# HKPolyU-UAV/bluerov2

Hardware: AMD Instinct MI355X
Metric: NMPC RTI solves/s (N=20, 12 states / 4 inputs), batch 4096 per GPU (higher is better)
Workload: dtype f64; 1 GPU; BASELINE.json configs[1]: batch=4096 independent BlueROV2 NMPC instances per GPU, N=20, Ts=0.05 s, circle reference window advancing one row per step, per-instance x0 noise (seed 1), nominal parameters, default options (qp_early_exit=1: exact equality-constrained shortcut when no bound is active); batch_per_gpu=4096, N=20, parallelism=single GPU

## Files before the change

bluerov2_amd/csrc/qp/fused.hpp:

```cpp
#pragma once

namespace brov {

constexpr int kFusedMaxN = 23;
template <int W, bool GRID, bool DF>
__device__ __forceinline__ bool rti_fused_step(const DevParams& P, int b, int lane, bool listed, size_t yoff) {
    extern __shared__ __attribute__((aligned(16))) double smem[];
    const int N = P.N;
    double* ba_s = smem;
    double* bv_s = ba_s + (size_t)N * kBaStage;
    double* kt_s = bv_s + (size_t)N * NX;
    double* kff_s = kt_s + (size_t)N * kKtStage;
    double* vh_s = kff_s + (size_t)N * 4;
    double* dx_s = vh_s + (size_t)N * 4;
    double* q_s = dx_s + (size_t)(N + 1) * NX;
    double* r_s = q_s + (size_t)(N + 1) * NX;
    double* const_s = r_s + (size_t)N * 4;
    if (lane == 0) { const_s[0] = 0.0; const_s[1] = 1.0; }
    LaneCst lc;
    if constexpr (W == 1) lc = load_lane_cst(P.cst, lane);
    double part = 0.0;
    bool nanp = false;
    lin_phase<W == 1, GRID>(P, b, 0, N, lane, ba_s, bv_s, kt_s, q_s, r_s, part, nanp, true, yoff);
    __syncthreads();
    if (P.dump_lin) copy_out_linearisation(P, b, 0, N, lane, ba_s, bv_s);
    std::conditional_t<GRID, InstGrid, Inst> I;
    setup_inst(P, I, b, lane, W == 1 ? &lc : nullptr, yoff);
    const bool listed_u = __builtin_amdgcn_readfirstlane((int)listed) != 0;
    I.ckpt = (N >= 8 && P.partial_refactor && listed_u) ? (N + 3) >> 2 : 0;
    I.lds_ba = (const lds_f64*)ba_s;
    I.lds_bv = (const lds_f64*)bv_s;
    I.lds_kt = (lds_f64*)kt_s;
    I.lds_q = (const lds_f64*)q_s;
    I.lds_r = (const lds_f64*)r_s;
    I.kff = kff_s;
    I.vhat = vh_s;
    I.dxb = dx_s;
    I.lds_kff = (lds_f64*)kff_s;
    I.lds_vhat = (lds_f64*)vh_s;
    I.lds_dxb = (lds_f64*)dx_s;
    I.lds_zero = (lds_f64*)const_s;
    I.lds_tr = (lds_f64*)const_s + 2;
    {
        const int rg = I.rg, cl = I.cl;
        const int zero = (int)(const_s - ba_s), one = zero + 1, kt0 = (int)(kt_s - ba_s);
        for (int r = 0; r < 3; r++) I.ba_off[r] = cl >= 3 ? (rg + 4 * r) * kBaStride + cl - 3 : ((r == 0 && rg == cl) ? one : zero);
        I.ba_str = cl >= 3 ? kBaStage : 0;
        for (int r = 0; r < 4; r++) {
            const int c = rg + 4 * r;
            I.bat_off[r] = cl >= NX ? zero : (c >= 3 ? cl * kBaStride + c - 3 : (c == cl ? one : zero));
        }
        I.bat_str = cl >= NX ? 0 : kBaStage;
        I.bat_str0 = (cl < NX && rg == 3) ? kBaStage : 0;
        for (int r = 0; r < 3; r++) I.kt_off[r] = cl < 4 ? kt0 + (rg + 4 * r) * 4 + cl : zero;
        I.kt_str = cl < 4 ? kKtStage : 0;
    }
    qp_body<W, std::conditional_t<GRID, InstGrid, Inst>, DF>(P, I, b, part, nanp);
    return I.ran_loop;
}
__device__ __forceinline__ void plant_step_wave(const DevParams& P, int b, int lane, int tk) {
    double x[NX], u[NU], k[NX], xs[NX], acc[NX];
    double* x0 = P.x0_rw + (size_t)b * NX;
#pragma unroll
    for (int j = 0; j < NX; j++) x[j] = x0[j];
#pragma unroll
    for (int j = 0; j < NU; j++) u[j] = P.res[b].u0[j];
    const ModelPar m = make_par(P.plant_pp + (size_t)b * NP);
    Wrench w = make_wrench(u);
    if (P.plant_rp) { w.k3 = P.plant_rp[(size_t)b * P.plant_rp_stride]; w.k4 = P.plant_rp[(size_t)b * P.plant_rp_stride + 1]; }
    const double h = P.plant_dt / P.plant_substeps;
    StagePoint sp;
    for (int s = 0; s < P.plant_substeps; s++) {
        model_f(x, w, m, NoWorldWrench{}, k, sp);
#pragma unroll
        for (int j = 0; j < NX; j++) { acc[j] = x[j] + (h / 6.0) * k[j]; xs[j] = x[j] + 0.5 * h * k[j]; }
        model_f(xs, w, m, NoWorldWrench{}, k, sp);
#pragma unroll
        for (int j = 0; j < NX; j++) { acc[j] += (h / 3.0) * k[j]; xs[j] = x[j] + 0.5 * h * k[j]; }
        model_f(xs, w, m, NoWorldWrench{}, k, sp);
#pragma unroll
        for (int j = 0; j < NX; j++) { acc[j] += (h / 3.0) * k[j]; xs[j] = x[j] + h * k[j]; }
        model_f(xs, w, m, NoWorldWrench{}, k, sp);
#pragma unroll
        for (int j = 0; j < NX; j++) x[j] = acc[j] + (h / 6.0) * k[j];
    }
    if (lane == 0) {
#pragma unroll
        for (int j = 0; j < NX; j++) x0[j] = x[j];
        if (P.plant_xlog) {
#pragma unroll
            for (int j = 0; j < NX; j++) P.plant_xlog[((size_t)tk * P.B + b) * NX + j] = x[j];
        }
        if (P.plant_ulog) {
#pragma unroll
            for (int j = 0; j < NU; j++) P.plant_ulog[((size_t)tk * P.B + b) * NU + j] = u[j];
        }
    }
}

template <int W, bool GRID = false, bool DF = false, bool MULTI = false>
__device__ __forceinline__ void rti_fused_body(const DevParams& P) {
    const int b = __builtin_amdgcn_readfirstlane(sched_map(P, blockIdx.x));
    const int lane = threadIdx.x;
    bool listed = sched_listed(P, b);
    if (blockIdx.x == 0) sched_zero_next(P, lane);
    DBG_STAMP(0);
    if constexpr (!MULTI) {
        (void)rti_fused_step<W, GRID, DF>(P, b, lane, listed, 0);
    } else {
#pragma clang loop unroll(disable)
        for (int tk = 0; tk < P.ticks; tk++) {
            int bq = b, lq = lane;
            asm volatile("s_mov_b32 %0, %0" : "+s"(bq));
            asm volatile("v_mov_b32 %0, %0" : "+v"(lq));
            listed = rti_fused_step<W, GRID, DF>(P, bq, lq, listed, (size_t)tk * (size_t)P.tick_yref);
            if (P.tick_status && lq == 0) P.tick_status[(size_t)tk * P.B + bq] = P.res[bq].status;
            __syncthreads();
            wave_fence();
            if (P.plant_pp) {
                plant_step_wave(P, bq, lq, tk);
                __syncthreads();
                wave_fence();
            }
        }
    }
}

}
```

bluerov2_amd/csrc/qp/lin_phase.hpp:

```cpp
#pragma once

namespace brov {

template <int MAXC>
__device__ __forceinline__ void stage_issue(const double* __restrict__ g, int nd, int lane, dbl2 (&v)[MAXC]) {
#pragma unroll
    for (int k = 0; k < MAXC; k++) {
        const int o = (lane + 64 * k) * 2;
        v[k] = *(const dbl2*)(g + (o < nd ? o : 0));
    }
}
template <int MAXC>
__device__ __forceinline__ void stage_store(double* l, int nd, int lane, const dbl2 (&v)[MAXC]) {
#pragma unroll
    for (int k = 0; k < MAXC; k++) {
        const int o = (lane + 64 * k) * 2;
        if (o < nd) *(lds_d2*)(l + o) = v[k];
    }
}

template <bool TWO = true, bool GRID = false>
__device__ __forceinline__ void lin_phase(const DevParams& P, int b, int i0, int n, int lane, double* ba_s, double* bv_s,
                                          double* rec_s, double* q_s, double* r_s, double& part, bool& nanp, bool stamp, size_t yoff = 0) {
#ifdef BROV_DBG_LIN
    unsigned long long lin_t[8] = {0, 0, 0, 0, 0, 0, 0, 0};
#endif
    const int N = P.N;
    const double* __restrict__ cst = P.cst;
    const int L = n <= 4 ? 16 : 64 / n;
    const int g = lane / L, j0 = lane - g * L;
    const bool active = g < n;
    const int i = active ? g : n - 1;
    const int ig = i0 + i;
    const double* __restrict__ ui = P.u + ((size_t)b * N + ig) * NU;
    const double hstep = GRID ? P.tsv[ig] : P.Ts;
    double rp0 = 0.0, rp1 = 0.0;
    if constexpr (TWO) {
        if (P.par_rp) { const double* rp = P.par_rp + ((size_t)b * (N + 1) + ig) * 2; rp0 = rp[0]; rp1 = rp[1]; }
    }
    const int po = i0 > 0 ? 1 : 0;
    double* sx = ba_s;
    double* spar = sx + (size_t)(n + 1) * NX;
    double* syr = spar + (size_t)n * NP;
    double* spi = syr + (size_t)(n + 1) * NY;
    double* su = spi + (size_t)(n + 1) * NX;
    {
        dbl2 vx[3], vp[3], vy[3], vpi[3], vu[1];
        stage_issue(P.x + ((size_t)b * (N + 1) + i0) * NX, (n + 1) * NX, lane, vx);
        stage_issue(P.par + ((size_t)b * (N + 1) + i0) * NP, n * NP, lane, vp);
        stage_issue(P.yref + yoff + (size_t)b * P.yref_stride + (size_t)i0 * NY, (n + 1) * NY, lane, vy);
        stage_issue(P.pi + ((size_t)b * N + i0 - po) * NX, (n + po) * NX, lane, vpi);
        stage_issue(P.u + ((size_t)b * N + i0) * NU, n * NU, lane, vu);
        stage_store(sx, (n + 1) * NX, lane, vx);
        stage_store(spar, n * NP, lane, vp);
        stage_store(syr, (n + 1) * NY, lane, vy);
        stage_store(spi, (n + po) * NX, lane, vpi);
        stage_store(su, n * NU, lane, vu);
    }
    const double* xi = sx + i * NX;
    const double* pp = spar + i * NP;
    const double* yr = syr + i * NY;
    const double* pil = spi + (i + po) * NX;
    const double* pim1 = spi + (ig > 0 ? i + po - 1 : 0) * NX;
    double uu[NU], x0r[NX], yrr[NY], pir[NX], pm1[3];
#pragma unroll
    for (int j = 0; j < NU; j++) uu[j] = su[i * NU + j];
#pragma unroll
    for (int j = 0; j < NX; j++) { x0r[j] = xi[j]; pir[j] = pil[j]; }
#pragma unroll
    for (int j = 0; j < NY; j++) yrr[j] = yr[j];
#pragma unroll
    for (int j = 0; j < 3; j++) pm1[j] = pim1[j];
    const unsigned long long tA = (stamp && P.dbg) ? __builtin_readcyclecounter() : 0;
    LIN_T(0);
    const bool last = ig == N - 1;
    double yrn[NX];
#pragma unroll
    for (int j = 0; j < NX; j++) yrn[j] = yr[NY + j];
    const ModelPar m = make_par(pp);
    Wrench w = make_wrench(uu);
    if constexpr (!TWO) {
        if (P.par_rp) { const double* rp = P.par_rp + ((size_t)b * (N + 1) + ig) * 2; rp0 = rp[0]; rp1 = rp[1]; }
    }
    w.k3 = rp0; w.k4 = rp1;
    KktAcc ka;
#pragma unroll
    for (int k = 0; k < NX; k++) {
        const double qk = (GRID ? P.wst[(size_t)ig * 16 + k] : P.Ts * cst[k]) * (x0r[k] - yrr[k]);
        q_s[i * NX + k] = qk;
        if (k < 3) ka.upd(ig >= 1 ? qk + pir[k] - pm1[k] : 0.0);
    }
#pragma unroll
    for (int k = 0; k < NU; k++) r_s[i * NU + k] = (GRID ? P.wst[(size_t)ig * 16 + NX + k] : P.Ts * cst[NX + k]) * (uu[k] - yrr[NX + k]);
    if (last) {
#pragma unroll
        for (int k = 0; k < NX; k++) {
            const double qn = cst[16 + k] * (xi[NX + k] - yrn[k]);
            q_s[n * NX + k] = qn;
            if (k < 3) ka.upd(qn - pir[k]);
        }
    }
    const unsigned long long tB = (stamp && P.dbg) ? __builtin_readcyclecounter() : 0;
    LIN_T(1);
    StagePoint sp[4];
    double xn[NX];
    rk4_state(x0r, w, m, hstep, sp, xn);
    const unsigned long long tC = (stamp && P.dbg) ? __builtin_readcyclecounter() : 0;
    LIN_T(2);
    double* tb = ba_s + i * kBaStage;
    lds_f64* rec = (lds_f64*)rec_s + i * kRecInterval;
#pragma unroll
    for (int st = 0; st < 4; st++) store_stage_rec(rec + st * kRecStage, sp[st], m);
#pragma unroll
    for (int k = 0; k < NX; k++) {
        const double bk = xn[k] - xi[NX + k];
        bv_s[i * NX + k] = bk;
        ka.upd(bk);
    }
    if (stamp && P.dbg && lane == 0)
        P.dbg[(size_t)b * 8 + 7] = ((tB - tA) & 0xFFFFF) | (((tC - tB) & 0xFFFFF) << 20) | (((__builtin_readcyclecounter() - tC) & 0xFFFFF) << 40);
    LIN_T(3);
    auto finish = [&](int c, const KktOperands& ko, const double (&acc)[NX]) __attribute__((always_inline)) {
        lin_kkt_col(ka, ko, N, ig, c, pir, acc);
#pragma unroll
        for (int k = 0; k < NX; k++) tb[k * kBaStride + (c - 3)] = acc[k];
    };
    if constexpr (TWO) {
#pragma unroll 1
        for (int q0 = j0; q0 - j0 < 6; q0 += 2 * L) {
            const int qa = q0 < 6 ? q0 : 5, qb = q0 + L < 6 ? q0 + L : 5;
            const int ca = qa < 3 ? 3 + qa : 6 + qa, cb = qb < 3 ? 3 + qb : 6 + qb;
            double acc0[NX], acc1[NX];
            const KktOperands koa = load_kkt_operands(P, cst, b, ig, i, n, ca, ui, (const lds_f64*)q_s, (const lds_f64*)r_s);
            const KktOperands kob = load_kkt_operands(P, cst, b, ig, i, n, cb, ui, (const lds_f64*)q_s, (const lds_f64*)r_s);
            sens_column_rec2(rec, m, hstep, ca, cb, acc0, acc1);
            finish(ca, koa, acc0);
            finish(cb, kob, acc1);
        }
    } else {
#pragma unroll 1
        for (int q0 = j0; q0 - j0 < 6; q0 += L) {
            const int qa = q0 < 6 ? q0 : 5;
            const int ca = qa < 3 ? 3 + qa : 6 + qa;
            double acc0[NX];
            const KktOperands koa = load_kkt_operands(P, cst, b, ig, i, n, ca, ui, (const lds_f64*)q_s, (const lds_f64*)r_s);
            sens_column_rec(rec, m, hstep, ca, acc0);
            finish(ca, koa, acc0);
        }
    }
    LIN_T(4);
    constexpr int kCheapTrips = 3;
    const int nC = (5 + L - 1) / L;
    KktGlobal kg[kCheapTrips];
    int cq[kCheapTrips];
#pragma unroll
    for (int t = 0; t < kCheapTrips; t++) {
        int q = j0 + t * L;
        q = q < 5 ? q : 4;
        cq[t] = q;
        const bool input = q >= 3;
        const int j = input ? (q == 3 ? 0 : 2) : q;
        kg[t] = load_kkt_global(P, b, ig, input ? NX + j : 6 + j, ui);
    }
#pragma unroll 1
    for (int q0 = j0; q0 - j0 < 2; q0 += L) {
        const int q = q0 < 2 ? q0 : 1;
        const int jc = 1 + 2 * q, c = NX + jc;
        double acc[NX];
        const KktOperands ko = load_kkt_operands(P, cst, b, ig, i, n, c, ui, (const lds_f64*)q_s, (const lds_f64*)r_s);
        sens_column_rec_u(rec, m, hstep, jc, acc);
        finish(c, ko, acc);
    }
    LIN_T(5);
    double cv[kCheapTrips][4];
#pragma unroll
    for (int t = 0; t < kCheapTrips; t++) {
        if (t < nC) {
            const int q = cq[t];
            const bool input = q >= 3;
            const int j = input ? (q == 3 ? 0 : 2) : q;
            constexpr double ir = 1.0 / kRotor;
            const double kbv = !input ? 0.0 : (j == 0 ? (-4.0 * 0.707) * ir * m.imx : -2.0 * ir * m.imz);
            sens_column_cheap(rec, hstep, j, input, kbv, cv[t]);
        }
    }
    LIN_T(6);
#pragma unroll
    for (int t = 0; t < kCheapTrips; t++) {
        if (t < nC) {
            const int q = cq[t];
            const bool input = q >= 3;
            const int j = input ? (q == 3 ? 0 : 2) : q;
            const int c = input ? NX + j : 6 + j;
            double acc[NX];
            expand_cheap(cv[t], j, acc);
            const double pr = (j == 0) ? pir[6] : ((j == 1) ? pir[7] : pir[8]);
            const double dotpi = cv[t][0] * pir[0] + cv[t][1] * pir[1] + cv[t][2] * pir[2] + cv[t][3] * pr;
            lin_kkt_rows(ka, finish_kkt_operands(kg[t], cst, i, n, c, (const lds_f64*)q_s, (const lds_f64*)r_s), N, ig, c, dotpi,
                         input ? 0.0 : pr);
#pragma unroll
            for (int k = 0; k < NX; k++) tb[k * kBaStride + (c - 3)] = acc[k];
        }
    }
    LIN_T(7);
#ifdef BROV_DBG_LIN
    if (stamp && P.dbg && lane == 0)
        for (int k = 0; k < 7; k++) P.dbg[(size_t)P.B * 8 + (size_t)b * 8 + (k == 6 ? 7 : k)] = lin_t[k + 1] - lin_t[k];
#endif
    if (active) {
        if (ka.nan) nanp = true;
        part = fmax(part, ka.mx);
    }
}

__device__ __forceinline__ void copy_out_linearisation(const DevParams& P, int b, int i0, int n, int lane, const double* ba_s,
                                                       const double* bv_s) {
    const int rg = lane >> 4, cl = lane & 15;
    const size_t g0 = (size_t)b * P.N + i0;
    for (int il = 0; il < n; il++) {
        const double* t = ba_s + il * kBaStage;
        double* BA = P.BA + (g0 + il) * 192;
#pragma unroll
        for (int r = 0; r < 3; r++) {
            const int row = rg + 4 * r;
            const double v = t[row * kBaStride + (cl >= 3 ? cl - 3 : 0)];
            const double m = cl >= 3 ? 1.0 : 0.0, c0 = (cl < 3 && row == cl) ? 1.0 : 0.0;
            BA[r * 64 + lane] = fma(m, v, c0);
        }
    }
    for (int j = lane; j < n * NX; j += 64) P.bvec[g0 * NX + j] = bv_s[j];
}

constexpr int kLinChunkMax = 21;
__host__ __device__ inline int lin_chunks(int N) { return (N + kLinChunkMax - 1) / kLinChunkMax; }
__host__ __device__ inline int lin_chunk_len(int N) { const int nc = lin_chunks(N); return (N + nc - 1) / nc; }
template <bool GRID>
__device__ __forceinline__ void lin_wave_body(const DevParams& P) {
    extern __shared__ __attribute__((aligned(16))) double lsm[];
    const int N = P.N, lane = threadIdx.x;
    const int nc = lin_chunks(N), C = lin_chunk_len(N);
    const int b = blockIdx.x / nc, ch = blockIdx.x - b * nc;
    const int i0 = ch * C;
    const int n = (N - i0 < C) ? N - i0 : C;
    double* ba_s = lsm;
    double* bv_s = ba_s + (size_t)C * kBaStage;
    double* rec_s = bv_s + (size_t)C * NX;
    double* q_s = rec_s + (size_t)C * kRecInterval;
    double* r_s = q_s + (size_t)(C + 1) * NX;
    double* part_s = r_s + (size_t)C * NU;
    double part = 0.0;
    bool nanp = false;
    lin_phase<true, GRID>(P, b, i0, n, lane, ba_s, bv_s, rec_s, q_s, r_s, part, nanp, false);
    part_s[lane] = nanp ? __builtin_nan("") : part;
    __syncthreads();
    const size_t g0 = (size_t)b * N + i0;
    copy_out_linearisation(P, b, i0, n, lane, ba_s, bv_s);
    {
        const int L = n <= 4 ? 16 : 64 / n;
        if (lane < n) {
            double m = 0.0;
            bool bad = false;
            for (int j = 0; j < L; j++) {
                const double v = part_s[lane * L + j];
                if (v != v) bad = true; else m = fmax(m, v);
            }
            P.kktp[g0 + lane] = bad ? __builtin_nan("") : m;
        }
    }
}

}
```

bluerov2_amd/csrc/qp/sched.hpp:

```cpp
#pragma once

namespace brov {

template <int MODE, int T>
struct IpmVec {
    double r[T];
    double* g;
    __device__ __forceinline__ double get(int t, int j) const { return MODE ? r[t % T] : g[j]; }
    __device__ __forceinline__ void set(int t, int j, double v) { if (MODE) r[t % T] = v; else g[j] = v; }
    __device__ __forceinline__ void fetch(int lane, int nv) {
        if constexpr (MODE == 2) {
#pragma unroll
            for (int t = 0; t < T; t++) { const unsigned j = (unsigned)lane + 64u * t; r[t] = g[j < (unsigned)nv ? j : 0u]; }
        }
    }
    __device__ __forceinline__ void flush(int lane, int nv) const {
        if constexpr (MODE == 2) {
#pragma unroll
            for (int t = 0; t < T; t++) { const unsigned j = (unsigned)lane + 64u * t; if (j < (unsigned)nv) g[j] = r[t]; }
        }
    }
};

constexpr int kSchedClasses = 64, kSchedCntStride = 32;
__host__ __device__ inline int sched_class_len(int B) { return (B + kSchedClasses - 1) / kSchedClasses; }
__host__ __device__ inline int sched_buffer_ints(int B) { return kSchedClasses * kSchedCntStride + kSchedClasses * sched_class_len(B) + B; }
__device__ __forceinline__ int sched_map(const DevParams& P, int t) {
    if (!P.sched) return t;
    const int32_t* __restrict__ Rd = P.sched + (size_t)P.sched_r * P.sched_stride;
    const int k = t & (kSchedClasses - 1), i = t >> 6, Bc = sched_class_len(P.B);
    const int n = Rd[k * kSchedCntStride];
    if (n <= 0 || 2 * n > Bc) return t;
    const int32_t* __restrict__ L = Rd + kSchedClasses * kSchedCntStride + k * Bc;
    const int32_t* __restrict__ pos = Rd + kSchedClasses * kSchedCntStride + kSchedClasses * Bc;
    if (i < n) return L[i];
    int x = pos[t];
    if (x < 0) return t;
    for (int guard = 0; guard < n; guard++) {
        const int y = pos[x * kSchedClasses + k];
        if (y < 0) break;
        x = y;
    }
    return x * kSchedClasses + k;
}
__device__ __forceinline__ const int32_t* uniform_ptr(const int32_t* p) {
    const unsigned long long v = (unsigned long long)p;
    const unsigned lo = __builtin_amdgcn_readfirstlane((unsigned)v), hi = __builtin_amdgcn_readfirstlane((unsigned)(v >> 32));
    return (const int32_t*)(((unsigned long long)hi << 32) | lo);
}
__device__ __forceinline__ int wave_atomic_inc(int32_t* addr_uniform) {
    int ret = 0;
    const int zero = 0, one = 1;
    unsigned long long saved;
    asm volatile(
        "s_mov_b64 %[sv], exec\n\t"
        "s_mov_b64 exec, 1\n\t"
        "global_atomic_add %[r], %[off], %[one], %[base] sc0\n\t"
        "s_waitcnt vmcnt(0)\n\t"
        "s_mov_b64 exec, %[sv]"
        : [r] "+v"(ret), [sv] "=&s"(saved)
        : [off] "v"(zero), [one] "v"(one), [base] "s"(addr_uniform)
        : "memory");
    return __builtin_amdgcn_readfirstlane(ret);
}
__device__ __forceinline__ int sched_ticket(const DevParams& P, int b) {
    if (!P.sched) return -1;
    int32_t* Wr = (int32_t*)uniform_ptr(P.sched + (size_t)P.sched_w * P.sched_stride);
    return wave_atomic_inc(Wr + (b & (kSchedClasses - 1)) * kSchedCntStride);
}
__device__ __forceinline__ void sched_note(const DevParams& P, int b, int p) {
    if (!P.sched) return;
    int32_t* Wr = (int32_t*)uniform_ptr(P.sched + (size_t)P.sched_w * P.sched_stride);
    const int Bc = sched_class_len(P.B), k = b & (kSchedClasses - 1);
    if (p >= 0 && p < Bc) Wr[kSchedClasses * kSchedCntStride + k * Bc + p] = b;
    Wr[kSchedClasses * kSchedCntStride + kSchedClasses * Bc + b] = p;
}
__device__ __forceinline__ bool sched_listed(const DevParams& P, int b) {
    if (!P.sched) return true;
    const int32_t* Rd = uniform_ptr(P.sched + (size_t)P.sched_r * P.sched_stride);
    return Rd[kSchedClasses * kSchedCntStride + kSchedClasses * sched_class_len(P.B) + b] >= 0;
}
__device__ __forceinline__ void sched_zero_next(const DevParams& P, int lane) {
    if (P.sched && lane < kSchedClasses) P.sched[(size_t)P.sched_z * P.sched_stride + lane * kSchedCntStride] = 0;
}

}
```

Before: 5.752 million solves/s.

## Speculatively prefetch stage data before resolving scheduler mapping in fused RTI kernel

The single-tick fused kernel now issues the global loads for the state, parameters, reference, multipliers and inputs of the block's own index before the scheduler lookup finishes. A hook inside lin_phase then settles the real instance index. If the scheduler remapped the block, it reissues the loads for the correct instance. This is meant to hide the dependent scheduler-table load chain behind the stage data fetch. It costs duplicate loads whenever the mapping differs and adds extra code paths, including debug timestamp writes.

```diff
diff --git a/bluerov2_amd/csrc/qp/fused.hpp b/bluerov2_amd/csrc/qp/fused.hpp
--- a/bluerov2_amd/csrc/qp/fused.hpp
+++ b/bluerov2_amd/csrc/qp/fused.hpp
@@ -3,8 +3,29 @@
 namespace brov {
 
 constexpr int kFusedMaxN = 23;
-template <int W, bool GRID, bool DF>
-__device__ __forceinline__ bool rti_fused_step(const DevParams& P, int b, int lane, bool listed, size_t yoff) {
+
+struct DbgEntry { unsigned long long cyc, rt, hw; };
+struct FusedHeadHook {
+    const DevParams& P;
+    int t, lane;
+    SchedHead& h;
+    const DbgEntry& de;
+    int& b_out;
+    __device__ __forceinline__ int operator()() const {
+        const int b = sched_head_settle(P, t, h);
+        b_out = b;
+        if (t == 0) sched_zero_next(P, lane);
+        if (P.dbg && lane == 0) {
+            P.dbg[(size_t)b * 8] = de.cyc;
+            P.dbg[(size_t)P.B * 8 + (size_t)b * 8 + 7] = de.rt;
+            P.dbg[(size_t)P.B * 8 + (size_t)b * 8 + 5] = de.hw;
+        }
+        return b;
+    }
+};
+
+template <int W, bool GRID, bool DF, bool HEAD>
+__device__ __forceinline__ bool rti_fused_step(const DevParams& P, int b, int lane, bool listed, SchedHead* head, const DbgEntry* de, size_t yoff) {
     extern __shared__ __attribute__((aligned(16))) double smem[];
     const int N = P.N;
     double* ba_s = smem;
@@ -21,12 +42,19 @@
     if constexpr (W == 1) lc = load_lane_cst(P.cst, lane);
     double part = 0.0;
     bool nanp = false;
-    lin_phase<W == 1, GRID>(P, b, 0, N, lane, ba_s, bv_s, kt_s, q_s, r_s, part, nanp, true, yoff);
+    if constexpr (HEAD) {
+        const int t = b;
+        lin_phase<W == 1, GRID>(P, t, 0, N, lane, ba_s, bv_s, kt_s, q_s, r_s, part, nanp, true, yoff, FusedHeadHook{P, t, lane, *head, *de, b});
+    } else {
+        lin_phase<W == 1, GRID>(P, b, 0, N, lane, ba_s, bv_s, kt_s, q_s, r_s, part, nanp, true, yoff);
+    }
     __syncthreads();
     if (P.dump_lin) copy_out_linearisation(P, b, 0, N, lane, ba_s, bv_s);
     std::conditional_t<GRID, InstGrid, Inst> I;
     setup_inst(P, I, b, lane, W == 1 ? &lc : nullptr, yoff);
-    const bool listed_u = __builtin_amdgcn_readfirstlane((int)listed) != 0;
+    bool listed_u;
+    if constexpr (HEAD) listed_u = __builtin_amdgcn_readfirstlane(head->raw) >= 0;
+    else listed_u = __builtin_amdgcn_readfirstlane((int)listed) != 0;
     I.ckpt = (N >= 8 && P.partial_refactor && listed_u) ? (N + 3) >> 2 : 0;
     I.lds_ba = (const lds_f64*)ba_s;
     I.lds_bv = (const lds_f64*)bv_s;
@@ -100,20 +128,28 @@
 
 template <int W, bool GRID = false, bool DF = false, bool MULTI = false>
 __device__ __forceinline__ void rti_fused_body(const DevParams& P) {
-    const int b = __builtin_amdgcn_readfirstlane(sched_map(P, blockIdx.x));
-    const int lane = threadIdx.x;
-    bool listed = sched_listed(P, b);
-    if (blockIdx.x == 0) sched_zero_next(P, lane);
-    DBG_STAMP(0);
     if constexpr (!MULTI) {
-        (void)rti_fused_step<W, GRID, DF>(P, b, lane, listed, 0);
+        const int lane = threadIdx.x;
+        DbgEntry de{0, 0, 0};
+        if (P.dbg) {
+            de.cyc = __builtin_readcyclecounter();
+            de.rt = __builtin_amdgcn_s_memrealtime();
+            de.hw = ((unsigned long long)__builtin_amdgcn_s_getreg(63508) << 32) | __builtin_amdgcn_s_getreg(63492);
+        }
+        SchedHead head = sched_head_issue(P, blockIdx.x);
+        (void)rti_fused_step<W, GRID, DF, true>(P, blockIdx.x, lane, true, &head, &de, 0);
     } else {
+        const int b = __builtin_amdgcn_readfirstlane(sched_map(P, blockIdx.x));
+        const int lane = threadIdx.x;
+        bool listed = sched_listed(P, b);
+        if (blockIdx.x == 0) sched_zero_next(P, lane);
+        DBG_STAMP(0);
 #pragma clang loop unroll(disable)
         for (int tk = 0; tk < P.ticks; tk++) {
             int bq = b, lq = lane;
             asm volatile("s_mov_b32 %0, %0" : "+s"(bq));
             asm volatile("v_mov_b32 %0, %0" : "+v"(lq));
-            listed = rti_fused_step<W, GRID, DF>(P, bq, lq, listed, (size_t)tk * (size_t)P.tick_yref);
+            listed = rti_fused_step<W, GRID, DF, false>(P, bq, lq, listed, nullptr, nullptr, (size_t)tk * (size_t)P.tick_yref);
             if (P.tick_status && lq == 0) P.tick_status[(size_t)tk * P.B + bq] = P.res[bq].status;
             __syncthreads();
             wave_fence();
diff --git a/bluerov2_amd/csrc/qp/lin_phase.hpp b/bluerov2_amd/csrc/qp/lin_phase.hpp
--- a/bluerov2_amd/csrc/qp/lin_phase.hpp
+++ b/bluerov2_amd/csrc/qp/lin_phase.hpp
@@ -19,9 +19,11 @@
     }
 }
 
-template <bool TWO = true, bool GRID = false>
+struct NoLinHook {};
+template <bool TWO = true, bool GRID = false, class Hook = NoLinHook>
 __device__ __forceinline__ void lin_phase(const DevParams& P, int b, int i0, int n, int lane, double* ba_s, double* bv_s,
-                                          double* rec_s, double* q_s, double* r_s, double& part, bool& nanp, bool stamp, size_t yoff = 0) {
+                                          double* rec_s, double* q_s, double* r_s, double& part, bool& nanp, bool stamp, size_t yoff = 0,
+                                          Hook hook = Hook{}) {
 #ifdef BROV_DBG_LIN
     unsigned long long lin_t[8] = {0, 0, 0, 0, 0, 0, 0, 0};
 #endif
@@ -51,6 +53,21 @@
         stage_issue(P.yref + yoff + (size_t)b * P.yref_stride + (size_t)i0 * NY, (n + 1) * NY, lane, vy);
         stage_issue(P.pi + ((size_t)b * N + i0 - po) * NX, (n + po) * NX, lane, vpi);
         stage_issue(P.u + ((size_t)b * N + i0) * NU, n * NU, lane, vu);
+        if constexpr (!std::is_same_v<Hook, NoLinHook>) {
+            const int bf = hook();
+            if (bf != b) {
+                b = bf;
+                ui = P.u + ((size_t)b * N + ig) * NU;
+                if constexpr (TWO) {
+                    if (P.par_rp) { const double* rp = P.par_rp + ((size_t)b * (N + 1) + ig) * 2; rp0 = rp[0]; rp1 = rp[1]; }
+                }
+                stage_issue(P.x + ((size_t)b * (N + 1) + i0) * NX, (n + 1) * NX, lane, vx);
+                stage_issue(P.par + ((size_t)b * (N + 1) + i0) * NP, n * NP, lane, vp);
+                stage_issue(P.yref + yoff + (size_t)b * P.yref_stride + (size_t)i0 * NY, (n + 1) * NY, lane, vy);
+                stage_issue(P.pi + ((size_t)b * N + i0 - po) * NX, (n + po) * NX, lane, vpi);
+                stage_issue(P.u + ((size_t)b * N + i0) * NU, n * NU, lane, vu);
+            }
+        }
         stage_store(sx, (n + 1) * NX, lane, vx);
         stage_store(spar, n * NP, lane, vp);
         stage_store(syr, (n + 1) * NY, lane, vy);
diff --git a/bluerov2_amd/csrc/qp/sched.hpp b/bluerov2_amd/csrc/qp/sched.hpp
--- a/bluerov2_amd/csrc/qp/sched.hpp
+++ b/bluerov2_amd/csrc/qp/sched.hpp
@@ -84,4 +84,49 @@
     if (P.sched && lane < kSchedClasses) P.sched[(size_t)P.sched_z * P.sched_stride + lane * kSchedCntStride] = 0;
 }
 
+struct SchedHead {
+    int n;
+    int raw;
+};
+__device__ __forceinline__ int sched_vload(const int32_t* base_uniform, unsigned idx) {
+    asm volatile("" : "+v"(idx));
+    return ((const __attribute__((address_space(1))) int32_t*)base_uniform)[idx];
 }
+__device__ __forceinline__ unsigned sched_pos_index(const DevParams& P, int b) {
+    return (unsigned)(kSchedClasses * kSchedCntStride + kSchedClasses * sched_class_len(P.B) + b);
+}
+__device__ __forceinline__ SchedHead sched_head_issue(const DevParams& P, int t) {
+    SchedHead h{0, 0};
+    if (P.sched) {
+        const int32_t* Rd = P.sched + (size_t)P.sched_r * P.sched_stride;
+        h.n = sched_vload(Rd, (unsigned)((t & (kSchedClasses - 1)) * kSchedCntStride));
+        h.raw = sched_vload(Rd, sched_pos_index(P, t));
+    }
+    return h;
+}
+__device__ __forceinline__ int sched_head_settle(const DevParams& P, int t, SchedHead& h) {
+    if (!P.sched) return t;
+    const int n = __builtin_amdgcn_readfirstlane(h.n), Bc = sched_class_len(P.B);
+    if (n <= 0 || 2 * n > Bc) return t;
+    const int32_t* __restrict__ Rd = P.sched + (size_t)P.sched_r * P.sched_stride;
+    const int k = t & (kSchedClasses - 1), i = t >> 6;
+    const int32_t* __restrict__ pos = Rd + kSchedClasses * kSchedCntStride + kSchedClasses * Bc;
+    int b;
+    if (i < n) {
+        b = Rd[kSchedClasses * kSchedCntStride + k * Bc + i];
+    } else {
+        int x = __builtin_amdgcn_readfirstlane(h.raw);
+        if (x < 0) return t;
+        for (int guard = 0; guard < n; guard++) {
+            const int y = pos[x * kSchedClasses + k];
+            if (y < 0) break;
+            x = y;
+        }
+        b = x * kSchedClasses + k;
+    }
+    b = __builtin_amdgcn_readfirstlane(b);
+    if (b != t) h.raw = sched_vload(Rd, sched_pos_index(P, b));
+    return b;
+}
+
+}
```

Result: no change. 5.744 million solves/s (-0.1%).
